# JTtNinjaCode/CPU-Ray-Tracing-Implementation

Measured on AMD Instinct MI355X. Metric: Msamples/sec (pixels*spp) Cornell Box 800x800@1024spp; 1/2/4/8-GPU scaling, higher is better.
Workload: dtype fp64; 1 GPU; cornell_box 800x800 1024spp depth 50, light sampling on; key=cornell_box 800x800 1024spp depth 50 f64 pool=0 chunk=0 K=0 world=1, spp=1024, max_depth=50, tiles=16x16 round-robin over ranks, parallelism=tiles1, kernel_timing=on, rounds_per_frame=1, grid_lanes=458752

## Files before the change

cpu-ray-tracing-implementation_amd/csrc/rt_plan.h:

```cpp
#pragma once

#include <stddef.h>
#include <stdint.h>

#include <algorithm>

#include "../../include/rt_hip.h"
#include "rt_scene.h"

namespace rtd {

inline void div_magic(uint32_t d, uint64_t& m, uint32_t& k) {
  uint32_t l = 0;
  while ((1ull << l) < d) l++;
  k = 32 + l;
  m = (uint64_t)((((unsigned __int128)1) << k) / d) + 1;
}

enum KernelFamily { KF_FLAT, KF_LIN_QUAD, KF_LIN_VOL, KF_LIN_SPH, KF_LIN_ALL, KF_WIDE, KF_STACK };
inline KernelFamily kernel_family(const SceneHeader& h, int32_t cam_mode, bool persist, bool ordered) {
  const bool persp = cam_mode == RT_CAM_PERSPECTIVE, procedural = h.n_texdata > 0 || h.has_cell_noise;
  const bool sph = h.n_spheres > 0, tri = h.n_tris > 0, vol = h.has_volumes != 0;
  if (!ordered && h.has_flat && persp && !procedural) return KF_FLAT;
  if (h.n_linear > 0) {
// ... 31 lines not shown
}
inline bool occlusion_early_exit(const SceneHeader& h, TraceFamily f, size_t word_bytes) {
  if (f != TF_LINEAR && f != TF_STACK) return true;
  if (h.has_volumes != 0) return false;
  if (f == TF_STACK && word_bytes == 16 && h.has_quads64 != 0) return false;
  return true;
}
inline KernelFamily trace_render_family(TraceFamily f) {
  return f == TF_FLAT ? KF_FLAT : f == TF_LINEAR ? KF_LIN_ALL : f == TF_STACK ? KF_STACK : KF_WIDE;
}
inline const char* trace_family_name(TraceFamily f) {
  static const char* n[] = {"flat program", "linear program", "wide BVH in LDS", "wide BVH in HBM", "binary BVH"};
  return n[f];
}

inline const char* family_name(KernelFamily f) {
  static const char* n[] = {"flat program", "linear program (quads)", "linear program (quads + volumes)",
                            "linear program (spheres)", "linear program (all kinds)", "wide BVH", "binary BVH"};
  return n[f];
}

inline bool lamb_light_scene(const SceneHeader& h) {
  const uint32_t ok_m = (1u << M_LAMBERTIAN) | (1u << M_DIFFUSE_LIGHT);
  return (h.mat_kinds & ~ok_m) == 0 && (h.tex_kinds & ~(1u << T_SOLID)) == 0 && h.light_kind == L_QUAD &&
         h.light_aligned != 0;
}
inline bool no_light_scene(const SceneHeader& h) {
  const uint32_t ok_m = (1u << M_LAMBERTIAN) | (1u << M_METAL) | (1u << M_DIELECTRIC);
  return (h.mat_kinds & ~ok_m) == 0 && (h.tex_kinds & ~((1u << T_SOLID) | (1u << T_CHECKER))) == 0 &&
         h.light_kind == L_NONE;
}
inline bool lamb_iso_light_scene(const SceneHeader& h) {
  const uint32_t ok_m = (1u << M_LAMBERTIAN) | (1u << M_DIFFUSE_LIGHT) | (1u << M_ISOTROPIC);
  return (h.mat_kinds & ~ok_m) == 0 && (h.tex_kinds & ~(1u << T_SOLID)) == 0 && h.light_kind == L_QUAD &&
         h.light_aligned != 0;
}

constexpr uint32_t kMaxItemsPerPixel = 256;
constexpr uint32_t kMinAutoChunk = 2;
struct PlanKnobs {
  uint32_t chunk = 8, chunk_flat = 32;
  uint32_t tail_chunk = 4, tail_chunk_flat = 8;
  double tail_frac = 0.5, tail_frac_flat = 0.125;
  uint64_t items_target = 4000000;
  uint64_t partial_budget = 2ull << 30;
};

struct ItemPlan {
  uint32_t chunk, tail_chunk, k_bulk, nchunks;
  uint32_t cpp;
  uint32_t passes;
  uint64_t partial_bytes;
};

inline ItemPlan plan_items(uint32_t spp, int32_t samples_per_item, bool flat, uint64_t full_pixels, uint32_t npix,
                           uint32_t elem, const PlanKnobs& kn) {
  const bool automatic = samples_per_item <= 0;
  uint32_t chunk0 = std::min(spp, automatic ? std::max(1u, flat ? kn.chunk_flat : kn.chunk) : (uint32_t)samples_per_item);
  if (automatic)
    while (chunk0 > kMinAutoChunk && full_pixels * ((spp + chunk0 - 1) / chunk0) < kn.items_target) chunk0 /= 2;
  ItemPlan pl{};
  pl.chunk = pl.tail_chunk = chunk0;
  pl.k_bulk = pl.nchunks = (spp + chunk0 - 1) / chunk0;
  if (automatic) {
    const double frac = std::min(1.0, std::max(0.0, flat ? kn.tail_frac_flat : kn.tail_frac));
    const uint32_t ts = std::min<uint32_t>(spp, (uint32_t)((double)spp * frac + 0.5));
    pl.tail_chunk = std::min(pl.chunk, std::max(1u, flat ? kn.tail_chunk_flat : kn.tail_chunk));
    for (;;) {
      pl.k_bulk = (spp - ts) / pl.chunk;
      pl.nchunks = pl.k_bulk + (spp - pl.k_bulk * pl.chunk + pl.tail_chunk - 1) / pl.tail_chunk;
      if (pl.nchunks <= kMaxItemsPerPixel || pl.chunk >= spp) break;
      pl.chunk = std::min(spp, 2 * pl.chunk);
      pl.tail_chunk = std::min(pl.chunk, 2 * pl.tail_chunk);
    }
  }
  const uint64_t per_chunk = 3ull * elem * npix;
  pl.cpp = (uint32_t)std::max<uint64_t>(
      1, std::min<uint64_t>({(uint64_t)pl.nchunks, kn.partial_budget / per_chunk, ((1ull << 31) - 1) / npix}));
  pl.passes = (pl.nchunks + pl.cpp - 1) / pl.cpp;
  pl.partial_bytes = per_chunk * pl.cpp;
  return pl;
}

}
```

cpu-ray-tracing-implementation_amd/csrc/rt_render.hip:

```cpp
#include <hip/hip_runtime.h>

#include <algorithm>
#include <chrono>
#include <cstdio>
#include <cstdlib>
#include <cstring>
#include <mutex>
#include <new>
#include <stdexcept>
#include <string>
#include <vector>

#include "../../include/rt_hip.h"
#include "rt_launch.h"
#include "rt_plan.h"
#include "scene_compile.h"

using namespace rtd;

struct DevBuf {
  void* ptr = nullptr;
  size_t bytes = 0;
};

struct rt_context {
  int device = 0;
  hipStream_t stream = nullptr;
  std::string err;
  CompiledScene scene;
  bool has_scene = false;
  DevBuf scene32, scene64;
  DevBuf state, partial, pixmap, queue0, queue1, blk, out_tmp, counters, camx, heads, tiles;
  DevBuf wide_spill;
  CamDev cam_host;
  uint32_t* total_host = nullptr;
  uint64_t samples = 0;
  rt_counters last{};
  int timing = 0;
  std::vector<hipEvent_t> events;
  hipStream_t pend_stream = nullptr;
  bool pending = false;
  size_t ev_used = 0;
  DevBuf fault;
  std::vector<uint4> tiles_dev;
  void* pixmap_for = nullptr;
  uint32_t pixmap_npix = 0;
  CamDev cam_dev{};
  bool cam_valid = false;
  bool scene_dirty32 = false, scene_dirty64 = false;
  DevBuf ids, q_rays, q_geom, q_ids;
  bool ids_dirty = false;
};

namespace {

CamDev make_view(const rt_camera_desc* c) {
  CamDev v{};
  v.mode = c->mode;
  double du[3], dv[3], dir00[3], pos00[3];
  for (int k = 0; k < 3; k++) {
    du[k] = (c->right[k] * c->viewport_width) / (double)c->image_width;
    dv[k] = (c->up[k] * -c->viewport_height) / (double)c->image_height;
  }
  for (int k = 0; k < 3; k++) {
    double a = c->dir[k] * c->focal_length;
    double b = c->right[k] * (c->viewport_width / 2.0);
    double u = c->up[k] * (c->viewport_height / 2.0);
    double e = (du[k] + dv[k]) * 0.5;
    dir00[k] = ((a - b) + u) + e;
    pos00[k] = ((c->pos[k] - b) + u) + e;
  }
  v.pos = {c->pos[0], c->pos[1], c->pos[2]};
  v.du = {du[0], du[1], du[2]};
  v.dv = {dv[0], dv[1], dv[2]};
  v.dir00 = {dir00[0], dir00[1], dir00[2]};
  v.pos00 = {pos00[0], pos00[1], pos00[2]};
  v.dir = {c->dir[0], c->dir[1], c->dir[2]};
  v.fdir = {c->focus_dist * c->dir[0], c->focus_dist * c->dir[1], c->focus_dist * c->dir[2]};
  v.disk_u = {c->defocus_u[0], c->defocus_u[1], c->defocus_u[2]};
  v.disk_v = {c->defocus_v[0], c->defocus_v[1], c->defocus_v[2]};
  v.focal = c->focal_length;
  return v;
}

std::mutex g_err_mu;
std::string g_create_err;

rt_status set_err(rt_context* c, rt_status s, const std::string& m) {
  if (c) {
    c->err = m;
  } else {
    std::lock_guard<std::mutex> lk(g_err_mu);
    g_create_err = m;
  }
  return s;
}

#define RT_HIP(ctx, call)                                                                   \
  do {                                                                                      \
    hipError_t e_ = (call);                                                                 \
    if (e_ != hipSuccess)                                                                   \
      return set_err((ctx), RT_ERR_HIP, std::string(#call) + ": " + hipGetErrorString(e_)); \
  } while (0)

rt_status ensure(rt_context* c, DevBuf& b, size_t bytes) {
  if (b.ptr && b.bytes >= bytes) return RT_OK;
  if (b.ptr) {
    if (c->pending) RT_HIP(c, hipStreamSynchronize(c->pend_stream));
    RT_HIP(c, hipFree(b.ptr));
    b.ptr = nullptr;
    b.bytes = 0;
  }
  size_t want = std::max<size_t>(bytes, 256);
  hipError_t e = hipMalloc(&b.ptr, want);
  if (e != hipSuccess) {
    b.ptr = nullptr;
    (void)hipGetLastError();
    return set_err(c, RT_ERR_OUT_OF_MEMORY,
                   "hipMalloc(" + std::to_string(want) + " bytes): " + hipGetErrorString(e));
  }
  b.bytes = want;
  return RT_OK;
}

hipEvent_t take_event(rt_context* c, size_t idx) {
  while (c->events.size() <= idx) {
    hipEvent_t e = nullptr;
    if (hipEventCreate(&e) != hipSuccess) return nullptr;
    c->events.push_back(e);
  }
  return c->events[idx];
}

rt_status settle(rt_context* c) {
  if (!c->pending) return RT_OK;
  c->pending = false;
  RT_HIP(c, hipStreamSynchronize(c->pend_stream));
  unsigned long long* shards = (unsigned long long*)(c->total_host + 16);
  RT_HIP(c, hipMemcpy(shards, c->counters.ptr, sizeof(unsigned long long) * kSegShards, hipMemcpyDeviceToHost));
  uint64_t segs = 0;
  for (int k = 0; k < kSegShards; k++) segs += shards[k];
  c->last.segments = segs;
  double ms = 0;
  for (size_t k = 0; k + 1 < c->ev_used; k += 2) {
    float a = 0;
    RT_HIP(c, hipEventElapsedTime(&a, c->events[k], c->events[k + 1]));
    ms += a;
  }
  c->ev_used = 0;
  c->last.step_ms += ms;
  uint32_t fault = 0;
  if (c->fault.ptr) RT_HIP(c, hipMemcpy(&fault, c->fault.ptr, 4, hipMemcpyDeviceToHost));
  if (fault) return set_err(c, RT_ERR_HIP, "a path did not finish (internal error)");
  return RT_OK;
}

template <class R>
DevScene<R> dev_scene(const SceneHeader& h, void* base) {
  auto at = [&](uint64_t off) { return (const unsigned char*)base + off; };
  DevScene<R> s{};
  s.quads = (const Quad<R>*)at(h.off_quads);
  s.spheres = (const Sphere<R>*)at(h.off_spheres);
  s.tris = (const Tri<R>*)at(h.off_tris);
  s.insts = (const Instance<R>*)at(h.off_instances);
  s.vols = (const Volume<R>*)at(h.off_volumes);
  s.nodes = (const Node<R>*)at(h.off_nodes);
  s.refs = (const uint32_t*)at(h.off_refs);
  s.mats = (const Material<R>*)at(h.off_mats);
  s.texs = (const Texture<R>*)at(h.off_texs);
  s.light = (const Light<R>*)at(h.off_light);
  s.lin = (const LinRec<R>*)at(h.off_linear);
  s.n_linear = h.n_linear;
  s.has_flat = (int32_t)h.has_flat;
  s.flatq = (const FlatQuadT<R>*)at(h.off_flat_quad);
  s.flatb = (const FlatBoxT<R>*)at(h.off_flat_box);
  for (int a = 0; a < 3; a++) s.n_flatq[a] = h.n_flat_quad[a];
  s.n_flatb = h.n_flat_box;
  s.n_flatr = h.n_flat_room;
  s.n_mats = h.n_mats;
  s.root = h.root;
  s.background = h.background;
  s.has_volumes = h.has_volumes;
  s.n_nodes = h.n_nodes;
  s.texdata = (const double*)at(h.off_texdata);
  s.images = (const uint8_t*)at(h.off_images);
  s.has_procedural = h.n_texdata > 0 || h.has_cell_noise;
  s.has_wide = (int32_t)h.has_wide;
  s.wnodes = (const WNode*)at(h.off_wnodes);
  s.wprims = (const typename WWord<R>::T*)at(h.off_wprims);
  s.n_wnodes = h.n_wnodes;
  s.n_wprim_words = h.n_wprim_words;
  s.wroot = h.wroot;
  s.wide_stack = h.wide_stack;
  s.wide_kinds = h.wide_kinds;
  s.wide_big = h.wide_big;
  s.wide_top = h.wide_top;
  s.wnodesh = h.has_wnodesh ? (const WNodeH*)at(h.off_wnodesh) : nullptr;
  s.quads64 = h.has_quads64 ? (const Quad<double>*)at(h.off_quads64) : nullptr;
  return s;
}

template <class R>
rt_status wide_spill_area(rt_context* c, const SceneHeader& hdr, DevScene<R>& sc) {
  const uint32_t wide_need = hdr.wide_stack;
  constexpr uint32_t kWideLdsStack = wide_lds_stack<R>();
  if (hdr.has_wide && wide_need > kWideLdsStack) {
    int ncu = 0;
    RT_HIP(c, hipDeviceGetAttribute(&ncu, hipDeviceAttributeMultiprocessorCount, c->device));
    const uint32_t lanes = (uint32_t)std::max(ncu, 1) * 2048u;
    rt_status s;
    if ((s = ensure(c, c->wide_spill, 4ull * (wide_need - kWideLdsStack) * lanes)) != RT_OK) return s;
    sc.wide_spill = (uint32_t*)c->wide_spill.ptr;
    sc.spill_lanes = lanes;
  }
  return RT_OK;
}

constexpr int kBatch = 16;
constexpr uint32_t kAutoPool32 = 1u << 21;
constexpr uint32_t kAutoPool64 = 1u << 19;
constexpr int kAutoSegments = 16;
constexpr uint32_t kAutoPersistLanes = 1u << 22;

PlanKnobs env_knobs() {
  auto num = [](const char* name, double dflt) {
    const char* v = std::getenv(name);
    return (v && *v) ? std::strtod(v, nullptr) : dflt;
  };
  PlanKnobs k;
  k.chunk = (uint32_t)num("RT_ITEM_CHUNK", k.chunk);
  k.chunk_flat = (uint32_t)num("RT_ITEM_CHUNK_FLAT", k.chunk_flat);
  k.tail_chunk = (uint32_t)num("RT_ITEM_TAIL_CHUNK", k.tail_chunk);
  k.tail_chunk_flat = (uint32_t)num("RT_ITEM_TAIL_CHUNK_FLAT", k.tail_chunk_flat);
  k.tail_frac = num("RT_ITEM_TAIL_FRAC", k.tail_frac);
  k.tail_frac_flat = num("RT_ITEM_TAIL_FRAC_FLAT", k.tail_frac_flat);
  k.items_target = (uint64_t)num("RT_ITEMS_TARGET", (double)k.items_target);
  k.partial_budget = (uint64_t)num("RT_PARTIAL_BUDGET", (double)k.partial_budget);
  return k;
}

struct StepKind {
  KernelFamily fam;
  bool ll, nl, lli;
  int stack;
};

template <class R>
rt_status timed_step(rt_context* c, const LaunchParams<R>& p, const StepKind& k, uint32_t grid, hipStream_t st) {
  hipEvent_t e0 = nullptr, e1 = nullptr;
  if (c->timing) {
    e0 = take_event(c, c->ev_used);
    e1 = take_event(c, c->ev_used + 1);
    if (!e0 || !e1) return set_err(c, RT_ERR_HIP, "hipEventCreate failed");
    RT_HIP(c, hipEventRecord(e0, st));
  }
  launch_step<R>(p, k.fam, k.ll, k.nl, k.lli, k.stack, grid, st);
  if (c->timing) {
    RT_HIP(c, hipEventRecord(e1, st));
    c->ev_used += 2;
  }
  c->last.launches++;
  c->last.iterations++;
  return RT_OK;
}

template <class R>
rt_status run_persistent(rt_context* c, const LaunchParams<R>& p, const StepKind& k, uint32_t grid, hipStream_t st) {
  RT_HIP(c, hipMemsetAsync(c->heads.ptr, 0, 4ull * kHeads * kHeadStride, st));
  rt_status s;
  if ((s = timed_step(c, p, k, grid, st)) != RT_OK) return s;
  RT_HIP(c, hipGetLastError());
  c->last.grid_lanes = last_grid_lanes();
  return RT_OK;
}

template <class R>
rt_status run_wavefront(rt_context* c, LaunchParams<R> p, const StepKind& k, uint32_t nblk_max, hipStream_t st) {
  const uint32_t P = p.P;
  p.queue = nullptr;
  p.n = P;
  launch_init<R>(p, nblk_max, st);
  c->last.launches++;
  uint32_t* qbuf[2] = {(uint32_t*)c->queue0.ptr, (uint32_t*)c->queue1.ptr};
  int qsel = 0;
  uint32_t* blk = (uint32_t*)c->blk.ptr;
  uint32_t* d_total = blk + nblk_max + 1;
  const uint64_t iter_cap =
      c->last.iterations + (((uint64_t)(p.n_items + P - 1) / P) * p.chunk * (uint64_t)p.max_depth + p.K - 1) / p.K + 4 * kBatch;
  for (;;) {
    if (c->last.iterations > iter_cap) return set_err(c, RT_ERR_HIP, "wavefront did not drain (internal error)");
    const uint32_t grid = (p.n + kBlock - 1) / kBlock;
    rt_status s;
    for (int b = 0; b < kBatch; b++)
      if ((s = timed_step(c, p, k, grid, st)) != RT_OK) return s;
    RT_HIP(c, hipGetLastError());
    launch_count(p.D, sizeof(R) == 8, p.queue, p.n, blk, d_total, st);
    c->last.launches += 2;
    RT_HIP(c, hipMemcpyAsync(c->total_host, d_total, 4, hipMemcpyDeviceToHost, st));
    RT_HIP(c, hipStreamSynchronize(st));
    const uint32_t alive = *c->total_host;
    if (alive == 0) return RT_OK;
    if (p.queue || alive * 2 <= P) {
      uint32_t* nq = qbuf[qsel];
      qsel ^= 1;
      launch_compact(p.D, sizeof(R) == 8, p.queue, p.n, blk, nq, st);
      c->last.launches++;
      p.queue = nq;
      p.n = alive;
    }
  }
}

std::vector<uint4> pack_tiles(const rt_tile* tiles, int32_t ntiles, uint64_t& npix) {
  std::vector<uint4> tl;
  tl.reserve(ntiles);
  npix = 0;
  for (int t = 0; t < ntiles; t++) {
    if (tiles[t].width == 0 || tiles[t].height == 0) continue;
    tl.push_back(make_uint4((uint32_t)tiles[t].x0, (uint32_t)tiles[t].y0, (uint32_t)tiles[t].width, (uint32_t)npix));
    npix += (uint64_t)tiles[t].width * (uint64_t)tiles[t].height;
  }
  return tl;
}

rt_status pixel_map(rt_context* c, const std::vector<uint4>& tl, uint32_t npix, hipStream_t st) {
  rt_status s;
  const size_t pixmap_bytes = c->pixmap.bytes;
  if ((s = ensure(c, c->pixmap, 4ull * npix)) != RT_OK) return s;
  if (c->pixmap.bytes != pixmap_bytes) c->tiles_dev.clear();
  const bool same_tiles = c->pixmap_for == c->pixmap.ptr && c->pixmap_npix == npix && c->tiles_dev.size() == tl.size() &&
                          std::memcmp(c->tiles_dev.data(), tl.data(), sizeof(uint4) * tl.size()) == 0;
  if (!same_tiles) {
    if ((s = ensure(c, c->tiles, sizeof(uint4) * tl.size())) != RT_OK) return s;
    c->tiles_dev = tl;
    c->pixmap_for = c->pixmap.ptr;
    c->pixmap_npix = npix;
    RT_HIP(c, hipMemcpyAsync(c->tiles.ptr, c->tiles_dev.data(), sizeof(uint4) * tl.size(), hipMemcpyHostToDevice, st));
    launch_pixmap((const uint4*)c->tiles.ptr, (uint32_t)tl.size(), npix, (uint32_t*)c->pixmap.ptr, st);
  }
  return RT_OK;
}

rt_status camera_view(rt_context* c, const rt_camera_desc* cam, hipStream_t st) {
  rt_status s;
  c->cam_host = make_view(cam);
  if ((s = ensure(c, c->camx, sizeof(CamDev))) != RT_OK) return s;
  if (!c->cam_valid || std::memcmp(&c->cam_dev, &c->cam_host, sizeof(CamDev)) != 0) {
    RT_HIP(c, hipMemcpyAsync(c->camx.ptr, &c->cam_host, sizeof(CamDev), hipMemcpyHostToDevice, st));
    c->cam_dev = c->cam_host;
    c->cam_valid = true;
  }
  return RT_OK;
}

template <class R>
rt_status render(rt_context* c, const rt_camera_desc* cam, const rt_render_params* prm, const rt_tile* tiles,
                 int32_t ntiles, void* out, int32_t out_dev, hipStream_t st) {
  const bool f64 = sizeof(R) == 8;
  const CompiledScene& cs = c->scene;
  const SceneHeader& hdr = f64 ? cs.hdr64 : cs.hdr;
  void* sbase = f64 ? c->scene64.ptr : c->scene32.ptr;
  bool& dirty = f64 ? c->scene_dirty64 : c->scene_dirty32;
  auto t0 = std::chrono::steady_clock::now();
  if (c->pending && c->pend_stream != st) RT_HIP(c, hipStreamSynchronize(c->pend_stream));
  if (dirty) {
    const std::vector<unsigned char>& blob = f64 ? cs.blob64 : cs.blob32;
    RT_HIP(c, hipMemcpyAsync(sbase, blob.data(), blob.size(), hipMemcpyHostToDevice, st));
    dirty = false;
    c->pending = true;
    c->pend_stream = st;
  }

  uint64_t npix64 = 0;
  const std::vector<uint4> tl = pack_tiles(tiles, ntiles, npix64);
  if (npix64 >= (1ull << 31)) return set_err(c, RT_ERR_INVALID_ARGUMENT, "too many pixels in one call");
  const uint32_t npix = (uint32_t)npix64;
  if (npix == 0) return RT_OK;
  const size_t out_elems = 3ull * npix;
  rt_status s;
  void* dout = out;
  if (!out_dev) {
    if ((s = ensure(c, c->out_tmp, out_elems * sizeof(R))) != RT_OK) return s;
    dout = c->out_tmp.ptr;
  }

  if (prm->max_depth <= 0) {
    launch_zero<R>((R*)dout, (uint64_t)out_elems, st);
  } else {
    const uint32_t spp = (uint32_t)prm->spp;
    const bool persist = prm->segments_per_launch <= 0;
    const StepKind kind{kernel_family(hdr, cam->mode, persist, prm->traversal == RT_TRAV_ORDERED), lamb_light_scene(hdr),
                        no_light_scene(hdr), lamb_iso_light_scene(hdr), cs.stack_need};
    if (!family_built(kind.fam))
      return set_err(c, RT_ERR_UNSUPPORTED,
                     std::string("this build (RT_DEV_ONLY) has no ") + family_name(kind.fam) + " kernels");
    const ItemPlan plan = plan_items(spp, prm->samples_per_item, kind.fam == KF_FLAT,
                                     (uint64_t)cam->image_width * (uint64_t)cam->image_height, npix, sizeof(R), env_knobs());
    const uint32_t n_items = npix * plan.cpp;
    uint32_t P = prm->pool_slots > 0 ? (uint32_t)prm->pool_slots
                 : persist       ? kAutoPersistLanes
                                 : (f64 ? kAutoPool64 : kAutoPool32);
    P = std::max<uint32_t>(1, std::min(P, n_items));
    const uint32_t nblk_max = (P + kBlock - 1) / kBlock;

    auto al = [](size_t x) { return (x + 255) & ~size_t(255); };
    const size_t r4 = al(sizeof(R4<R>) * (size_t)P), sb = al(16 * (size_t)P), xb = al(16 * (size_t)P);
    if (!persist) {
      if ((s = ensure(c, c->state, 5 * r4 + sb + xb)) != RT_OK) return s;
      if ((s = ensure(c, c->queue0, 4ull * P)) != RT_OK) return s;
      if ((s = ensure(c, c->queue1, 4ull * P)) != RT_OK) return s;
    }
    if ((s = ensure(c, c->partial, plan.partial_bytes)) != RT_OK) return s;
    c->last.passes += plan.passes;
    c->last.partial_bytes = plan.partial_bytes;
    if ((s = ensure(c, c->blk, 4ull * (nblk_max + 2))) != RT_OK) return s;
    if ((s = pixel_map(c, tl, npix, st)) != RT_OK) return s;

    unsigned char* sp = (unsigned char*)c->state.ptr;
    LaunchParams<R> p{};
    p.sc = dev_scene<R>(hdr, sbase);
    if ((s = wide_spill_area<R>(c, hdr, p.sc)) != RT_OK) return s;
    if (prm->traversal == RT_TRAV_ORDERED) p.sc.has_flat = p.sc.has_wide = 0;
    p.sc.cam64 = nullptr;
    p.O = (R4<R>*)sp;
    p.D = (R4<R>*)(sp + r4);
    p.T = (R4<R>*)(sp + 2 * r4);
    p.L = (R4<R>*)(sp + 3 * r4);
    p.A = (R4<R>*)(sp + 4 * r4);
    p.S = (uint4*)(sp + 5 * r4);
    p.X = (uint4*)(sp + 5 * r4 + sb);
    p.partial = (R*)c->partial.ptr;
    p.pixmap = (const uint32_t*)c->pixmap.ptr;
    p.queue = nullptr;
    p.n = P;
    p.P = P;
    p.npix = npix;
    div_magic(npix, p.npix_m, p.npix_k);
    p.n_items = n_items;
    p.chunk = plan.chunk;
    p.k_bulk = plan.k_bulk;
    p.tail_chunk = plan.tail_chunk;
    p.spp = spp;
    p.first_sample = (uint32_t)std::max(0, prm->first_sample);
    p.W = (uint32_t)cam->image_width;
    p.max_depth = prm->max_depth;
    p.seed = prm->seed;
    if ((s = camera_view(c, cam, st)) != RT_OK) return s;
    p.cam_mode = c->cam_host.mode;
    p.camx = (const CamDev*)c->camx.ptr;
    if (p.cam_mode == RT_CAM_PERSPECTIVE) p.sc.cam64 = p.camx;
    p.seg_shards = (unsigned long long*)c->counters.ptr;
    p.K = prm->segments_per_launch > 0 ? std::min(prm->segments_per_launch, 64) : kAutoSegments;
    if (c->timing && c->ev_used > 4096 && (s = settle(c)) != RT_OK) return s;
    if (persist) {
      if ((s = ensure(c, c->fault, 4)) != RT_OK) return s;
      p.persist = kPersist;
      p.fault = (uint32_t*)c->fault.ptr;
      if ((s = ensure(c, c->heads, 4ull * kHeads * kHeadStride)) != RT_OK) return s;
      p.heads = (uint32_t*)c->heads.ptr;
    }
    for (uint32_t c0 = 0; c0 < plan.nchunks; c0 += plan.cpp) {
      const uint32_t pc = std::min(plan.cpp, plan.nchunks - c0);
      p.chunk0 = c0;
      p.n_items = npix * pc;
      s = persist ? run_persistent(c, p, kind, nblk_max, st) : run_wavefront(c, p, kind, nblk_max, st);
      if (s != RT_OK) return s;
      launch_resolve<R>((const R*)c->partial.ptr, npix, pc, spp, (R*)dout, c0 == 0, c0 + pc >= plan.nchunks, st);
      c->last.launches++;
      RT_HIP(c, hipGetLastError());
    }
    c->pending = true;
    c->pend_stream = st;
    c->last.samples += (uint64_t)npix * spp;
  }
  if (!out_dev) {
    RT_HIP(c, hipMemcpyAsync(out, dout, out_elems * sizeof(R), hipMemcpyDeviceToHost, st));
    RT_HIP(c, hipStreamSynchronize(st));
    if ((s = settle(c)) != RT_OK) return s;
  }
  c->last.last_render_ms = std::chrono::duration<double, std::milli>(std::chrono::steady_clock::now() - t0).count();
  return RT_OK;
}

rt_status query_scene(rt_context* c, bool f64, hipStream_t st) {
  const CompiledScene& cs = c->scene;
  bool& dirty = f64 ? c->scene_dirty64 : c->scene_dirty32;
  if (c->pending && c->pend_stream != st) RT_HIP(c, hipStreamSynchronize(c->pend_stream));
  if (dirty) {
    const std::vector<unsigned char>& blob = f64 ? cs.blob64 : cs.blob32;
    RT_HIP(c, hipMemcpyAsync(f64 ? c->scene64.ptr : c->scene32.ptr, blob.data(), blob.size(), hipMemcpyHostToDevice, st));
    dirty = false;
    c->pending = true;
    c->pend_stream = st;
  }
  if (c->ids_dirty) {
    if (!cs.ids.empty())
      RT_HIP(c, hipMemcpyAsync(c->ids.ptr, cs.ids.data(), cs.ids.size() * sizeof(int32_t), hipMemcpyHostToDevice, st));
    c->ids_dirty = false;
    c->pending = true;
    c->pend_stream = st;
  }
  return RT_OK;
}

template <class R>
rt_status trace_rays(rt_context* c, const rt_trace_params* prm, const double* rays, uint32_t n, double* geom,
                     int32_t* ids, hipStream_t st) {
  const bool f64 = sizeof(R) == 8;
  const CompiledScene& cs = c->scene;
  const SceneHeader& hdr = f64 ? cs.hdr64 : cs.hdr;
  void* sbase = f64 ? c->scene64.ptr : c->scene32.ptr;
  const bool ordered = prm->traversal == RT_TRAV_ORDERED;
  const TraceFamily fam = trace_family(hdr, ordered, sizeof(typename WWord<R>::T));
  if (!family_built(trace_render_family(fam)))
    return set_err(c, RT_ERR_UNSUPPORTED,
                   std::string("this build (RT_DEV_ONLY) has no ") + trace_family_name(fam) + " query kernel");
  rt_status s;
  if ((s = query_scene(c, f64, st)) != RT_OK) return s;
  TraceParams<R> p{};
  p.rays = rays;
  p.geom = geom;
  p.ids = ids;
  if (!prm->on_device) {
    if ((s = ensure(c, c->q_rays, 64ull * n)) != RT_OK) return s;
    if ((s = ensure(c, c->q_geom, 56ull * n)) != RT_OK) return s;
    if ((s = ensure(c, c->q_ids, 16ull * n)) != RT_OK) return s;
    RT_HIP(c, hipMemcpyAsync(c->q_rays.ptr, rays, 64ull * n, hipMemcpyHostToDevice, st));
    p.rays = (const double*)c->q_rays.ptr;
    p.geom = (double*)c->q_geom.ptr;
    p.ids = (int32_t*)c->q_ids.ptr;
  }
  p.sc = dev_scene<R>(hdr, sbase);
  if (fam == TF_WIDE_HBM && (s = wide_spill_area<R>(c, hdr, p.sc)) != RT_OK) return s;
  if (ordered) p.sc.has_flat = p.sc.has_wide = 0;
  p.sc.cam64 = nullptr;
  p.idtab = (const int2*)c->ids.ptr;
  for (int k = 0; k < 4; k++) p.id_off[k] = cs.ids_off[k];
  p.n = n;
  p.seed = prm->seed;
  p.seg_shards = (unsigned long long*)c->counters.ptr;
  launch_trace<R>(p, fam, st);
  RT_HIP(c, hipGetLastError());
  c->last.launches++;
  c->pending = true;
  c->pend_stream = st;
  if (!prm->on_device) {
    RT_HIP(c, hipMemcpyAsync(geom, p.geom, 56ull * n, hipMemcpyDeviceToHost, st));
    RT_HIP(c, hipMemcpyAsync(ids, p.ids, 16ull * n, hipMemcpyDeviceToHost, st));
    RT_HIP(c, hipStreamSynchronize(st));
    if ((s = settle(c)) != RT_OK) return s;
  }
  return RT_OK;
}

template <class R>
rt_status occluded(rt_context* c, const rt_trace_params* prm, const double* rays, uint32_t n, uint8_t* out,
                   hipStream_t st) {
  const bool f64 = sizeof(R) == 8;
  const CompiledScene& cs = c->scene;
  const SceneHeader& hdr = f64 ? cs.hdr64 : cs.hdr;
  void* sbase = f64 ? c->scene64.ptr : c->scene32.ptr;
  const bool ordered = prm->traversal == RT_TRAV_ORDERED;
  const TraceFamily fam = trace_family(hdr, ordered, sizeof(typename WWord<R>::T));
  if (!family_built(trace_render_family(fam)))
    return set_err(c, RT_ERR_UNSUPPORTED,
                   std::string("this build (RT_DEV_ONLY) has no ") + trace_family_name(fam) + " occlusion kernel");
  rt_status s;
  if ((s = query_scene(c, f64, st)) != RT_OK) return s;
  OcclParams<R> p{};
  p.rays = rays;
  p.out = out;
  if (!prm->on_device) {
    if ((s = ensure(c, c->q_rays, 64ull * n)) != RT_OK) return s;
    if ((s = ensure(c, c->q_ids, n)) != RT_OK) return s;
    RT_HIP(c, hipMemcpyAsync(c->q_rays.ptr, rays, 64ull * n, hipMemcpyHostToDevice, st));
    p.rays = (const double*)c->q_rays.ptr;
    p.out = (uint8_t*)c->q_ids.ptr;
  }
  p.sc = dev_scene<R>(hdr, sbase);
  if (fam == TF_WIDE_HBM && (s = wide_spill_area<R>(c, hdr, p.sc)) != RT_OK) return s;
  if (ordered) p.sc.has_flat = p.sc.has_wide = 0;
  p.sc.cam64 = nullptr;
  p.n = n;
  p.seed = prm->seed;
  p.seg_shards = (unsigned long long*)c->counters.ptr;
  launch_occluded<R>(p, fam, occlusion_early_exit(hdr, fam, sizeof(typename WWord<R>::T)), st);
  RT_HIP(c, hipGetLastError());
  c->last.launches++;
  c->pending = true;
  c->pend_stream = st;
  if (!prm->on_device) {
    RT_HIP(c, hipMemcpyAsync(out, p.out, n, hipMemcpyDeviceToHost, st));
    RT_HIP(c, hipStreamSynchronize(st));
    if ((s = settle(c)) != RT_OK) return s;
  }
  return RT_OK;
}

rt_status camera_rays(rt_context* c, const rt_camera_desc* cam, uint64_t seed, int32_t first_sample, uint32_t spp,
                      const std::vector<uint4>& tl, uint32_t npix, double* out, bool on_device, hipStream_t st) {
  rt_status s;
  if (c->pending && c->pend_stream != st) RT_HIP(c, hipStreamSynchronize(c->pend_stream));
  if ((s = pixel_map(c, tl, npix, st)) != RT_OK) return s;
  if ((s = camera_view(c, cam, st)) != RT_OK) return s;
  const uint64_t n = (uint64_t)npix * spp;
  CamRayParams p{};
  p.pixmap = (const uint32_t*)c->pixmap.ptr;
  p.camx = (const CamDev*)c->camx.ptr;
  p.rays = out;
  if (!on_device) {
    if ((s = ensure(c, c->q_rays, 64ull * n)) != RT_OK) return s;
    p.rays = (double*)c->q_rays.ptr;
  }
  p.npix = npix;
  p.spp = spp;
  p.first_sample = (uint32_t)std::max(0, first_sample);
  p.W = (uint32_t)cam->image_width;
  p.cam_mode = c->cam_host.mode;
  p.seed = seed;
  launch_camera_rays(p, st);
  RT_HIP(c, hipGetLastError());
  c->pending = true;
  c->pend_stream = st;
  if (!on_device) {
    RT_HIP(c, hipMemcpyAsync(out, p.rays, 64ull * n, hipMemcpyDeviceToHost, st));
    RT_HIP(c, hipStreamSynchronize(st));
    if ((s = settle(c)) != RT_OK) return s;
  }
  return RT_OK;
}

template <class R>
rt_status render_aov(rt_context* c, const rt_camera_desc* cam, const rt_aov_params* prm, const std::vector<uint4>& tl,
                     uint32_t npix, double* feat, int32_t* ids, hipStream_t st) {
  const bool f64 = sizeof(R) == 8;
  const CompiledScene& cs = c->scene;
  const SceneHeader& hdr = f64 ? cs.hdr64 : cs.hdr;
  const bool ordered = prm->traversal == RT_TRAV_ORDERED;
  const TraceFamily fam = aov_family(hdr, ordered, sizeof(typename WWord<R>::T));
  if (!family_built(trace_render_family(fam)))
    return set_err(c, RT_ERR_UNSUPPORTED,
                   std::string("this build (RT_DEV_ONLY) has no ") + trace_family_name(fam) + " feature-buffer kernel");
  rt_status s;
  if ((s = query_scene(c, f64, st)) != RT_OK) return s;
  if ((s = pixel_map(c, tl, npix, st)) != RT_OK) return s;
  if ((s = camera_view(c, cam, st)) != RT_OK) return s;
  AovParams<R> p{};
  p.feat = feat;
  p.ids = ids;
  if (!prm->on_device) {
    if ((s = ensure(c, c->q_geom, 64ull * npix)) != RT_OK) return s;
    if ((s = ensure(c, c->q_ids, 16ull * npix)) != RT_OK) return s;
    p.feat = (double*)c->q_geom.ptr;
    p.ids = (int32_t*)c->q_ids.ptr;
  }
  p.sc = dev_scene<R>(hdr, f64 ? c->scene64.ptr : c->scene32.ptr);
  if (fam == TF_WIDE_HBM && (s = wide_spill_area<R>(c, hdr, p.sc)) != RT_OK) return s;
  if (fam != TF_FLAT) p.sc.has_flat = 0;
  if (ordered) p.sc.has_wide = 0;
  p.sc.cam64 = nullptr;
  p.pixmap = (const uint32_t*)c->pixmap.ptr;
  p.camx = (const CamDev*)c->camx.ptr;
  p.idtab = (const int2*)c->ids.ptr;
  for (int k = 0; k < 4; k++) p.id_off[k] = cs.ids_off[k];
  p.npix = npix;
  p.spp = (uint32_t)prm->spp;
  p.first_sample = (uint32_t)std::max(0, prm->first_sample);
  p.W = (uint32_t)cam->image_width;
  p.cam_mode = c->cam_host.mode;
  p.ext = aov_extended(hdr, p.cam_mode) ? 1 : 0;
  p.seed = prm->seed;
  p.seg_shards = (unsigned long long*)c->counters.ptr;
  launch_aov<R>(p, fam, st);
  RT_HIP(c, hipGetLastError());
  c->last.launches++;
  c->pending = true;
  c->pend_stream = st;
  if (!prm->on_device) {
    RT_HIP(c, hipMemcpyAsync(feat, p.feat, 64ull * npix, hipMemcpyDeviceToHost, st));
    RT_HIP(c, hipMemcpyAsync(ids, p.ids, 16ull * npix, hipMemcpyDeviceToHost, st));
    RT_HIP(c, hipStreamSynchronize(st));
    if ((s = settle(c)) != RT_OK) return s;
  }
  return RT_OK;
}

rt_status check_camera_tiles(rt_context* c, const rt_camera_desc* cam, const rt_tile* tiles, int32_t ntiles) {
  if (cam->mode < RT_CAM_PERSPECTIVE || cam->mode > RT_CAM_LENS)
    return set_err(c, RT_ERR_INVALID_ARGUMENT, "unknown camera mode");
  if (cam->image_width <= 0 || cam->image_height <= 0) return set_err(c, RT_ERR_INVALID_ARGUMENT, "empty image");
  if (cam->image_width > 65535 || cam->image_height > 65535)
    return set_err(c, RT_ERR_INVALID_ARGUMENT, "image wider or taller than 65535 pixels");
  for (int t = 0; t < ntiles; t++) {
    const rt_tile& tl = tiles[t];
    if (tl.x0 < 0 || tl.y0 < 0 || tl.width < 0 || tl.height < 0 || tl.x0 + tl.width > cam->image_width ||
        tl.y0 + tl.height > cam->image_height)
      return set_err(c, RT_ERR_INVALID_ARGUMENT, "tile " + std::to_string(t) + " outside the image");
  }
  return RT_OK;
}

}


extern "C" {

int32_t rt_abi_version(void) { return RT_ABI_VERSION; }

#define RT_STR2(x) #x
#define RT_STR(x) RT_STR2(x)
const char* rt_build_info(void) {
  return "dev_only=" RT_STR(RT_DEV_ONLY) " wide_top_n=" RT_STR(RT_WIDE_TOP_N) " wide_lds_stack=" RT_STR(RT_WIDE_LDS_STACK) " wide_waves_global=" RT_STR(RT_WIDE_WAVES_GLOBAL)
#ifdef RT_SECTION_CLOCKS
      " sections=1"
#endif
#ifdef RT_DEBUG_TRACE
      " trace=1"
#endif
#ifdef RT_PRECISE_F32
      " precise_f32=1"
#endif
      ;
}
#undef RT_STR
#undef RT_STR2

rt_status rt_context_create(int32_t device, rt_context** out) {
  if (!out) return set_err(nullptr, RT_ERR_INVALID_ARGUMENT, "out is null");
  *out = nullptr;
  int n = 0;
  hipError_t e = hipGetDeviceCount(&n);
  if (e != hipSuccess || n == 0) {
    (void)hipGetLastError();
    return set_err(nullptr, RT_ERR_NO_DEVICE, std::string("no HIP device: ") + hipGetErrorString(e));
  }
  if (device < 0 || device >= n) return set_err(nullptr, RT_ERR_INVALID_ARGUMENT, "device index out of range");
  if ((e = hipSetDevice(device)) != hipSuccess) return set_err(nullptr, RT_ERR_HIP, hipGetErrorString(e));
  if ((e = upload_sincos_table()) != hipSuccess)
    return set_err(nullptr, RT_ERR_HIP, std::string("sin/cos table: ") + hipGetErrorString(e));
  auto* c = new rt_context;
  c->device = device;
  if ((e = hipStreamCreateWithFlags(&c->stream, hipStreamNonBlocking)) != hipSuccess) {
    delete c;
    return set_err(nullptr, RT_ERR_HIP, hipGetErrorString(e));
  }
  if ((e = hipHostMalloc((void**)&c->total_host, 64 + 8 * kSegShards, hipHostMallocDefault)) != hipSuccess) {
    (void)hipStreamDestroy(c->stream);
    delete c;
    return set_err(nullptr, RT_ERR_HIP, hipGetErrorString(e));
  }
  if (ensure(c, c->counters, sizeof(unsigned long long) * kSegShards) != RT_OK || ensure(c, c->fault, 4) != RT_OK ||
      hipMemset(c->counters.ptr, 0, sizeof(unsigned long long) * kSegShards) != hipSuccess ||
      hipMemset(c->fault.ptr, 0, 4) != hipSuccess) {
    std::string m = c->err;
    rt_context_destroy(c);
    return set_err(nullptr, RT_ERR_OUT_OF_MEMORY, m);
  }
  *out = c;
  return RT_OK;
}

void rt_context_destroy(rt_context* c) {
  if (!c) return;
  (void)hipSetDevice(c->device);
  if (c->pending) (void)hipStreamSynchronize(c->pend_stream);
  if (c->stream) (void)hipStreamSynchronize(c->stream);
  for (DevBuf* b : {&c->scene32, &c->scene64, &c->state, &c->partial, &c->pixmap, &c->queue0, &c->queue1, &c->blk, &c->wide_spill,
                    &c->out_tmp, &c->counters, &c->camx, &c->heads, &c->tiles, &c->fault, &c->ids, &c->q_rays, &c->q_geom,
                    &c->q_ids})
    if (b->ptr) (void)hipFree(b->ptr);
  for (hipEvent_t e : c->events) (void)hipEventDestroy(e);
  if (c->total_host) (void)hipHostFree(c->total_host);
  if (c->stream) (void)hipStreamDestroy(c->stream);
  delete c;
}

const char* rt_last_error(const rt_context* c) {
  if (c) return c->err.c_str();
  std::lock_guard<std::mutex> lk(g_err_mu);
  return g_create_err.c_str();
}

rt_status rt_scene_upload(rt_context* c, const rt_scene_desc* desc) {
  if (!c || !desc) return set_err(c, RT_ERR_INVALID_ARGUMENT, "null context or descriptor");
  RT_HIP(c, hipSetDevice(c->device));
  CompiledScene cs;
  std::string err;
  rt_status s = compile_scene(desc, &cs, &err);
  if (s != RT_OK) return set_err(c, s, err);
  if (c->pending) RT_HIP(c, hipStreamSynchronize(c->pend_stream));
  if ((s = ensure(c, c->scene32, cs.blob32.size())) != RT_OK) return s;
  if ((s = ensure(c, c->scene64, cs.blob64.size())) != RT_OK) return s;
  if ((s = ensure(c, c->ids, cs.ids.size() * sizeof(int32_t))) != RT_OK) return s;
  c->scene = std::move(cs);
  c->scene_dirty32 = c->scene_dirty64 = true;
  c->ids_dirty = true;
  c->has_scene = true;
  return RT_OK;
}

rt_status rt_scene_check(const rt_scene_desc* desc, rt_scene_info* info, char* err, int32_t errlen) {
  CompiledScene cs;
  std::string m;
  rt_status s = desc ? compile_scene(desc, &cs, &m) : RT_ERR_INVALID_ARGUMENT;
  if (!desc) m = "null descriptor";
  if (s == RT_OK) {
    const KernelFamily fam = kernel_family(cs.hdr, RT_CAM_PERSPECTIVE, true, false);
    if (!family_built(fam)) {
      s = RT_ERR_UNSUPPORTED;
      m = std::string("this build (RT_DEV_ONLY) has no ") + family_name(fam) + " kernels";
    }
  }
  if (err && errlen > 0) std::snprintf(err, (size_t)errlen, "%s", m.c_str());
  if (s == RT_OK && info) {
    const SceneHeader& h = cs.hdr;
    info->quads = cs.desc_quads;
    info->flat_quads = cs.flat_quads;
    info->flat_boxes = cs.flat_boxes;
    info->wide_nodes = cs.hdr.has_wide ? (int32_t)cs.hdr.n_wnodes : 0;
    info->wide_stack = cs.hdr.has_wide ? (int32_t)cs.hdr.wide_stack : 0;
    info->wide_kinds = cs.hdr.has_wide ? (int32_t)cs.hdr.wide_kinds : 0;
    info->wide_prim_words = cs.hdr.has_wide ? (int32_t)cs.hdr.n_wprim_words : 0;
    info->wide_big = cs.hdr.has_wide ? (int32_t)cs.hdr.wide_big : 0;
    info->spheres = (int32_t)h.n_spheres;
    info->triangles = (int32_t)h.n_tris;
    info->instances = h.num_instances;
    info->volumes = (int32_t)h.n_volumes;
    info->bvh_nodes = (int32_t)h.n_nodes;
    info->linear_ops = (int32_t)h.n_linear;
    info->stack_need = cs.stack_need;
    info->bytes_f32 = cs.blob32.size();
    info->bytes_f64 = cs.blob64.size();
  }
  return s;
}

rt_status rt_render_tiles(rt_context* c, const rt_camera_desc* cam, const rt_render_params* prm, const rt_tile* tiles,
                          int32_t ntiles, void* out_rgb, int32_t out_is_device, void* stream) {
  if (!c) return set_err(nullptr, RT_ERR_INVALID_ARGUMENT, "null context");
  if (!cam || !prm || (!tiles && ntiles > 0) || ntiles < 0 || (!out_rgb && ntiles > 0))
    return set_err(c, RT_ERR_INVALID_ARGUMENT, "null argument");
  if (!c->has_scene) return set_err(c, RT_ERR_NO_SCENE, "rt_scene_upload has not succeeded on this context");
  if (cam->mode < RT_CAM_PERSPECTIVE || cam->mode > RT_CAM_LENS)
    return set_err(c, RT_ERR_INVALID_ARGUMENT, "unknown camera mode");
  if (cam->image_width <= 0 || cam->image_height <= 0) return set_err(c, RT_ERR_INVALID_ARGUMENT, "empty image");
  if (cam->image_width > 65535 || cam->image_height > 65535)
    return set_err(c, RT_ERR_INVALID_ARGUMENT, "image wider or taller than 65535 pixels");
  if (prm->spp <= 0) return set_err(c, RT_ERR_INVALID_ARGUMENT, "spp must be positive");
  if (prm->precision != RT_PREC_F32 && prm->precision != RT_PREC_F64)
    return set_err(c, RT_ERR_INVALID_ARGUMENT, "unknown precision");
  for (int t = 0; t < ntiles; t++) {
    const rt_tile& tl = tiles[t];
    if (tl.x0 < 0 || tl.y0 < 0 || tl.width < 0 || tl.height < 0 || tl.x0 + tl.width > cam->image_width ||
        tl.y0 + tl.height > cam->image_height)
      return set_err(c, RT_ERR_INVALID_ARGUMENT, "tile " + std::to_string(t) + " outside the image");
  }
  RT_HIP(c, hipSetDevice(c->device));
  hipStream_t st = (stream == nullptr && !out_is_device) ? c->stream : (hipStream_t)stream;
  try {
    if (prm->precision == RT_PREC_F64) return render<double>(c, cam, prm, tiles, ntiles, out_rgb, out_is_device, st);
    return render<float>(c, cam, prm, tiles, ntiles, out_rgb, out_is_device, st);
  } catch (const std::bad_alloc&) {
    return set_err(c, RT_ERR_OUT_OF_MEMORY, "out of host memory");
  } catch (const std::exception& e) {
    return set_err(c, RT_ERR_INVALID_ARGUMENT, e.what());
  }
}

rt_status rt_trace_rays(rt_context* c, const rt_trace_params* prm, const double* rays, int64_t nrays, double* out_geom,
                        int32_t* out_ids, void* stream) {
  if (!c) return set_err(nullptr, RT_ERR_INVALID_ARGUMENT, "null context");
  if (!prm || !rays || !out_geom || !out_ids) return set_err(c, RT_ERR_INVALID_ARGUMENT, "null argument");
  if (nrays < 0 || nrays >= (1ll << 31)) return set_err(c, RT_ERR_INVALID_ARGUMENT, "nrays outside [0, 2^31)");
// ... 133 lines not shown
```

Measured before the change: 28140 Msamples/s.

## Overlap successive persistent render launches across two streams with double-buffered partials

Adds a second stream and a second set of partial and heads buffers, so consecutive persistent render launches alternate between lanes. Each launch can overlap the previous resolve and render, with events guarding input uploads and buffer reuse. The goal is to hide the serial gaps and tail effects between frames or chunk passes. It costs extra memory and synchronization logic, and the per-step timing subtracts the overlapping lead when launches on different lanes overlap.

```diff
diff --git a/cpu-ray-tracing-implementation_amd/csrc/rt_plan.h b/cpu-ray-tracing-implementation_amd/csrc/rt_plan.h
--- a/cpu-ray-tracing-implementation_amd/csrc/rt_plan.h
+++ b/cpu-ray-tracing-implementation_amd/csrc/rt_plan.h
@@ -137,4 +137,38 @@
   return pl;
 }
 
+struct LaneQuery {
+  bool knob;
+  bool device_out;
+  bool persist;
+  bool shared_scratch;
+  bool second_set;
+  uint64_t n;
+  bool inputs_written;
+  bool prev_overlapped;
+  bool lane_stale[2];
+  bool pending;
+  const void* caller;
+  const void* prev;
+};
+struct LanePlan {
+  bool overlap;
+  int lane, set;
+  bool sync_prev;
+  bool wait_resolve;
+  bool record_inputs;
+  bool wait_inputs;
+};
+inline LanePlan lane_plan(const LaneQuery& q) {
+  LanePlan pl{};
+  pl.sync_prev = q.pending && q.prev != q.caller;
+  pl.overlap = q.knob && q.device_out && q.persist && !q.shared_scratch && q.second_set;
+  if (!pl.overlap) return pl;
+  pl.lane = pl.set = (int)(q.n & 1);
+  pl.wait_resolve = q.n >= 2;
+  pl.record_inputs = q.inputs_written || !q.prev_overlapped;
+  pl.wait_inputs = pl.record_inputs || q.lane_stale[pl.lane];
+  return pl;
 }
+
+}
diff --git a/cpu-ray-tracing-implementation_amd/csrc/rt_render.hip b/cpu-ray-tracing-implementation_amd/csrc/rt_render.hip
--- a/cpu-ray-tracing-implementation_amd/csrc/rt_render.hip
+++ b/cpu-ray-tracing-implementation_amd/csrc/rt_render.hip
@@ -50,6 +50,18 @@
   bool scene_dirty32 = false, scene_dirty64 = false;
   DevBuf ids, q_rays, q_geom, q_ids;
   bool ids_dirty = false;
+  hipStream_t lane1 = nullptr;
+  DevBuf partial2, heads2;
+  hipEvent_t ev_done[2] = {nullptr, nullptr};
+  hipEvent_t ev_resolved[2] = {nullptr, nullptr};
+  hipEvent_t ev_inputs = nullptr;
+  bool lanes_failed = false;
+  uint64_t lane_launches = 0;
+  bool lanes_live = false;
+  bool inputs_written = false;
+  bool prev_overlapped = false;
+  bool lane_stale[2] = {false, false};
+  std::vector<uint8_t> ev_lane;
 };
 
 namespace {
@@ -103,10 +115,21 @@
       return set_err((ctx), RT_ERR_HIP, std::string(#call) + ": " + hipGetErrorString(e_)); \
   } while (0)
 
+rt_status wait_pending(rt_context* c) {
+  if (c->pending) RT_HIP(c, hipStreamSynchronize(c->pend_stream));
+  if (c->lanes_live) {
+    RT_HIP(c, hipStreamSynchronize(c->stream));
+    if (c->lane1) RT_HIP(c, hipStreamSynchronize(c->lane1));
+    c->lanes_live = false;
+  }
+  return RT_OK;
+}
+
 rt_status ensure(rt_context* c, DevBuf& b, size_t bytes) {
   if (b.ptr && b.bytes >= bytes) return RT_OK;
   if (b.ptr) {
-    if (c->pending) RT_HIP(c, hipStreamSynchronize(c->pend_stream));
+    rt_status w;
+    if ((w = wait_pending(c)) != RT_OK) return w;
     RT_HIP(c, hipFree(b.ptr));
     b.ptr = nullptr;
     b.bytes = 0;
@@ -134,8 +157,11 @@
 
 rt_status settle(rt_context* c) {
   if (!c->pending) return RT_OK;
+  {
+    rt_status w;
+    if ((w = wait_pending(c)) != RT_OK) return w;
+  }
   c->pending = false;
-  RT_HIP(c, hipStreamSynchronize(c->pend_stream));
   unsigned long long* shards = (unsigned long long*)(c->total_host + 16);
   RT_HIP(c, hipMemcpy(shards, c->counters.ptr, sizeof(unsigned long long) * kSegShards, hipMemcpyDeviceToHost));
   uint64_t segs = 0;
@@ -145,9 +171,17 @@
   for (size_t k = 0; k + 1 < c->ev_used; k += 2) {
     float a = 0;
     RT_HIP(c, hipEventElapsedTime(&a, c->events[k], c->events[k + 1]));
+    if (k >= 2 && k / 2 < c->ev_lane.size() && c->ev_lane[k / 2]) {
+      float lead = 0;
+      if (hipEventElapsedTime(&lead, c->events[k], c->events[k - 1]) == hipSuccess && lead > 0)
+        a = std::max(0.0f, a - lead);
+      else
+        (void)hipGetLastError();
+    }
     ms += a;
   }
   c->ev_used = 0;
+  c->ev_lane.clear();
   c->last.step_ms += ms;
   uint32_t fault = 0;
   if (c->fault.ptr) RT_HIP(c, hipMemcpy(&fault, c->fault.ptr, 4, hipMemcpyDeviceToHost));
@@ -239,6 +273,11 @@
   return k;
 }
 
+bool env_frame_overlap() {
+  const char* v = std::getenv("RT_FRAME_OVERLAP");
+  return !(v && *v) || std::strtol(v, nullptr, 10) != 0;
+}
+
 struct StepKind {
   KernelFamily fam;
   bool ll, nl, lli;
@@ -246,7 +285,8 @@
 };
 
 template <class R>
-rt_status timed_step(rt_context* c, const LaunchParams<R>& p, const StepKind& k, uint32_t grid, hipStream_t st) {
+rt_status timed_step(rt_context* c, const LaunchParams<R>& p, const StepKind& k, uint32_t grid, hipStream_t st,
+                     bool on_lane = false) {
   hipEvent_t e0 = nullptr, e1 = nullptr;
   if (c->timing) {
     e0 = take_event(c, c->ev_used);
@@ -257,6 +297,8 @@
   launch_step<R>(p, k.fam, k.ll, k.nl, k.lli, k.stack, grid, st);
   if (c->timing) {
     RT_HIP(c, hipEventRecord(e1, st));
+    c->ev_lane.resize(c->ev_used / 2 + 1, 0);
+    c->ev_lane[c->ev_used / 2] = on_lane;
     c->ev_used += 2;
   }
   c->last.launches++;
@@ -265,10 +307,11 @@
 }
 
 template <class R>
-rt_status run_persistent(rt_context* c, const LaunchParams<R>& p, const StepKind& k, uint32_t grid, hipStream_t st) {
-  RT_HIP(c, hipMemsetAsync(c->heads.ptr, 0, 4ull * kHeads * kHeadStride, st));
+rt_status run_persistent(rt_context* c, const LaunchParams<R>& p, const StepKind& k, uint32_t grid, hipStream_t st,
+                         bool on_lane = false) {
+  RT_HIP(c, hipMemsetAsync(p.heads, 0, 4ull * kHeads * kHeadStride, st));
   rt_status s;
-  if ((s = timed_step(c, p, k, grid, st)) != RT_OK) return s;
+  if ((s = timed_step(c, p, k, grid, st, on_lane)) != RT_OK) return s;
   RT_HIP(c, hipGetLastError());
   c->last.grid_lanes = last_grid_lanes();
   return RT_OK;
@@ -335,6 +378,7 @@
     c->tiles_dev = tl;
     c->pixmap_for = c->pixmap.ptr;
     c->pixmap_npix = npix;
+    c->inputs_written = true;
     RT_HIP(c, hipMemcpyAsync(c->tiles.ptr, c->tiles_dev.data(), sizeof(uint4) * tl.size(), hipMemcpyHostToDevice, st));
     launch_pixmap((const uint4*)c->tiles.ptr, (uint32_t)tl.size(), npix, (uint32_t*)c->pixmap.ptr, st);
   }
@@ -346,11 +390,30 @@
   c->cam_host = make_view(cam);
   if ((s = ensure(c, c->camx, sizeof(CamDev))) != RT_OK) return s;
   if (!c->cam_valid || std::memcmp(&c->cam_dev, &c->cam_host, sizeof(CamDev)) != 0) {
+    c->inputs_written = true;
     RT_HIP(c, hipMemcpyAsync(c->camx.ptr, &c->cam_host, sizeof(CamDev), hipMemcpyHostToDevice, st));
     c->cam_dev = c->cam_host;
     c->cam_valid = true;
   }
   return RT_OK;
+}
+
+bool lanes_ready(rt_context* c, size_t partial_bytes) {
+  if (c->lanes_failed) return false;
+  if (!c->lane1) {
+    bool ok = hipStreamCreateWithFlags(&c->lane1, hipStreamNonBlocking) == hipSuccess;
+    for (hipEvent_t* e : {&c->ev_done[0], &c->ev_done[1], &c->ev_resolved[0], &c->ev_resolved[1], &c->ev_inputs})
+      ok = ok && hipEventCreateWithFlags(e, hipEventDisableTiming) == hipSuccess;
+    if (!ok) {
+      (void)hipGetLastError();
+      c->lanes_failed = true;
+      return false;
+    }
+  }
+  const std::string err = c->err;
+  const bool ok = ensure(c, c->heads2, 4ull * kHeads * kHeadStride) == RT_OK && ensure(c, c->partial2, partial_bytes) == RT_OK;
+  if (!ok) c->err = err;
+  return ok;
 }
 
 template <class R>
@@ -362,9 +425,18 @@
   void* sbase = f64 ? c->scene64.ptr : c->scene32.ptr;
   bool& dirty = f64 ? c->scene_dirty64 : c->scene_dirty32;
   auto t0 = std::chrono::steady_clock::now();
-  if (c->pending && c->pend_stream != st) RT_HIP(c, hipStreamSynchronize(c->pend_stream));
+  LaneQuery lq{};
+  lq.pending = c->pending;
+  lq.caller = (const void*)st;
+  lq.prev = (const void*)c->pend_stream;
+  if (lane_plan(lq).sync_prev) {
+    rt_status w;
+    if ((w = wait_pending(c)) != RT_OK) return w;
+    lq.pending = false;
+  }
   if (dirty) {
     const std::vector<unsigned char>& blob = f64 ? cs.blob64 : cs.blob32;
+    c->inputs_written = true;
     RT_HIP(c, hipMemcpyAsync(sbase, blob.data(), blob.size(), hipMemcpyHostToDevice, st));
     dirty = false;
     c->pending = true;
@@ -459,13 +531,59 @@
       if ((s = ensure(c, c->heads, 4ull * kHeads * kHeadStride)) != RT_OK) return s;
       p.heads = (uint32_t*)c->heads.ptr;
     }
+    lq.knob = env_frame_overlap();
+    lq.device_out = out_dev != 0;
+    lq.persist = persist;
+    lq.shared_scratch = p.sc.wide_spill != nullptr;
+    lq.second_set = true;
+    lq.second_set = lane_plan(lq).overlap && lanes_ready(c, plan.partial_bytes);
     for (uint32_t c0 = 0; c0 < plan.nchunks; c0 += plan.cpp) {
       const uint32_t pc = std::min(plan.cpp, plan.nchunks - c0);
       p.chunk0 = c0;
       p.n_items = npix * pc;
-      s = persist ? run_persistent(c, p, kind, nblk_max, st) : run_wavefront(c, p, kind, nblk_max, st);
-      if (s != RT_OK) return s;
-      launch_resolve<R>((const R*)c->partial.ptr, npix, pc, spp, (R*)dout, c0 == 0, c0 + pc >= plan.nchunks, st);
+      lq.n = c->lane_launches;
+      lq.inputs_written = c->inputs_written;
+      lq.prev_overlapped = c->prev_overlapped;
+      lq.lane_stale[0] = c->lane_stale[0];
+      lq.lane_stale[1] = c->lane_stale[1];
+      const LanePlan lp = lane_plan(lq);
+      const R* partial = (const R*)c->partial.ptr;
+      if (lp.overlap) {
+        hipStream_t lane = lp.lane ? c->lane1 : c->stream;
+        if (lp.set) {
+          p.partial = (R*)c->partial2.ptr;
+          p.heads = (uint32_t*)c->heads2.ptr;
+        } else {
+          p.partial = (R*)c->partial.ptr;
+          p.heads = (uint32_t*)c->heads.ptr;
+        }
+        partial = p.partial;
+        c->pending = true;
+        c->pend_stream = st;
+        c->lanes_live = true;
+        if (lp.wait_resolve) RT_HIP(c, hipStreamWaitEvent(lane, c->ev_resolved[lp.set], 0));
+        if (lp.record_inputs) {
+          RT_HIP(c, hipEventRecord(c->ev_inputs, st));
+          c->inputs_written = false;
+          c->lane_stale[0] = c->lane_stale[1] = true;
+        }
+        if (lp.wait_inputs) {
+          RT_HIP(c, hipStreamWaitEvent(lane, c->ev_inputs, 0));
+          c->lane_stale[lp.lane] = false;
+        }
+        c->prev_overlapped = true;
+        c->lane_launches++;
+        if ((s = run_persistent(c, p, kind, nblk_max, lane, true)) != RT_OK) return s;
+        RT_HIP(c, hipEventRecord(c->ev_done[lp.lane], lane));
+        RT_HIP(c, hipStreamWaitEvent(st, c->ev_done[lp.lane], 0));
+      } else {
+        c->prev_overlapped = false;
+        c->inputs_written = false;
+        s = persist ? run_persistent(c, p, kind, nblk_max, st) : run_wavefront(c, p, kind, nblk_max, st);
+        if (s != RT_OK) return s;
+      }
+      launch_resolve<R>(partial, npix, pc, spp, (R*)dout, c0 == 0, c0 + pc >= plan.nchunks, st);
+      if (lp.overlap) RT_HIP(c, hipEventRecord(c->ev_resolved[lp.set], st));
       c->last.launches++;
       RT_HIP(c, hipGetLastError());
     }
@@ -485,9 +603,11 @@
 rt_status query_scene(rt_context* c, bool f64, hipStream_t st) {
   const CompiledScene& cs = c->scene;
   bool& dirty = f64 ? c->scene_dirty64 : c->scene_dirty32;
-  if (c->pending && c->pend_stream != st) RT_HIP(c, hipStreamSynchronize(c->pend_stream));
+  rt_status s0;
+  if (c->pending && c->pend_stream != st && (s0 = wait_pending(c)) != RT_OK) return s0;
   if (dirty) {
     const std::vector<unsigned char>& blob = f64 ? cs.blob64 : cs.blob32;
+    c->inputs_written = true;
     RT_HIP(c, hipMemcpyAsync(f64 ? c->scene64.ptr : c->scene32.ptr, blob.data(), blob.size(), hipMemcpyHostToDevice, st));
     dirty = false;
     c->pending = true;
@@ -600,7 +720,7 @@
 rt_status camera_rays(rt_context* c, const rt_camera_desc* cam, uint64_t seed, int32_t first_sample, uint32_t spp,
                       const std::vector<uint4>& tl, uint32_t npix, double* out, bool on_device, hipStream_t st) {
   rt_status s;
-  if (c->pending && c->pend_stream != st) RT_HIP(c, hipStreamSynchronize(c->pend_stream));
+  if (c->pending && c->pend_stream != st && (s = wait_pending(c)) != RT_OK) return s;
   if ((s = pixel_map(c, tl, npix, st)) != RT_OK) return s;
   if ((s = camera_view(c, cam, st)) != RT_OK) return s;
   const uint64_t n = (uint64_t)npix * spp;
@@ -765,7 +885,11 @@
   (void)hipSetDevice(c->device);
   if (c->pending) (void)hipStreamSynchronize(c->pend_stream);
   if (c->stream) (void)hipStreamSynchronize(c->stream);
-  for (DevBuf* b : {&c->scene32, &c->scene64, &c->state, &c->partial, &c->pixmap, &c->queue0, &c->queue1, &c->blk, &c->wide_spill,
+  if (c->lane1) (void)hipStreamSynchronize(c->lane1);
+  for (hipEvent_t e : {c->ev_done[0], c->ev_done[1], c->ev_resolved[0], c->ev_resolved[1], c->ev_inputs})
+    if (e) (void)hipEventDestroy(e);
+  if (c->lane1) (void)hipStreamDestroy(c->lane1);
+  for (DevBuf* b : {&c->partial2, &c->heads2, &c->scene32, &c->scene64, &c->state, &c->partial, &c->pixmap, &c->queue0, &c->queue1, &c->blk, &c->wide_spill,
                     &c->out_tmp, &c->counters, &c->camx, &c->heads, &c->tiles, &c->fault, &c->ids, &c->q_rays, &c->q_geom,
                     &c->q_ids})
     if (b->ptr) (void)hipFree(b->ptr);
@@ -788,7 +912,7 @@
   std::string err;
   rt_status s = compile_scene(desc, &cs, &err);
   if (s != RT_OK) return set_err(c, s, err);
-  if (c->pending) RT_HIP(c, hipStreamSynchronize(c->pend_stream));
+  if ((s = wait_pending(c)) != RT_OK) return s;
   if ((s = ensure(c, c->scene32, cs.blob32.size())) != RT_OK) return s;
   if ((s = ensure(c, c->scene64, cs.blob64.size())) != RT_OK) return s;
   if ((s = ensure(c, c->ids, cs.ids.size() * sizeof(int32_t))) != RT_OK) return s;
```

Measured after the change: 28530 Msamples/s (median of 6 runs). 1.01x the previous value.
